# CrystalSixone/VLN-MAGIC

Hardware: AMD Instinct MI355X
Metric: trajectory-steps/sec (whole node), MAGIC-S R2R pretrain (higher is better)
Workload: dtype bf16

## Files before the change

### include/magic_hip.h

```cpp
#ifndef MAGIC_HIP_H
#define MAGIC_HIP_H
#ifdef __cplusplus
extern "C" {
#endif

#define MAGIC_OK 0
#define MAGIC_ERR_ARG (-1)
#define MAGIC_ERR_LAUNCH (-2)
#define MAGIC_ERR_UNSUPPORTED (-3)

int magic_abi_version(void);
int magic_build_id(char* out, int len);
int magic_device_info(int* cu_count, int* clock_khz, char* arch, int arch_len);

int magic_gemm(int dtype, int layout, int batch, int nh, int M, int N, int K,
               const void* A, int lda, long long sAb, long long sAh,
               const void* B, int ldb, long long sBb, long long sBh,
               void* C, int ldc, long long sCb, long long sCh, int c_f32, int accumulate,
               const float* bias, int epilogue, const void* aux, int ldaux,
               const void* residual, int ldr, void* C2, int ldc2,
               float alpha, int splitk, float* bias_grad, void* stream);
int magic_gemm_set_big(int mode);
#define MAGIC_GEMM_FORM_PLAIN 0x1
#define MAGIC_GEMM_FORM_XCD 0x2
// ... 184 lines not shown
int magic_mlm_eval_ws_need(int dtype, int nm, int V, int H);
int magic_mlm_eval(int dtype, int nm, int V, int H, const void* hm, const void* W, int ldw, const float* bias,
                   const int* labels, int ignore_index, void* ws, float* loss_row, int* hit_row, void* stream);
int magic_eval_rows(int dtype, int M, int N, const void* logits, int ld, const int* labels, int ignore_index,
                    const float* targets, int ldt, float* loss_row, int* hit_row, void* stream);
int magic_cfp_eval(int dtype, int B, int H, const void* a, const void* txt, float temperature,
                   float* loss_row, int* hit_row, void* stream);
int magic_eval_accum(int M, const float* loss_row, const int* hit_row, void* acc, int slot, void* stream);

int magic_csr_gather(int dtype, int n_out, int H, const void* src, const int* ptr, const int* idx, const float* w,
                     void* out, int accumulate, void* stream);
int magic_pano_fuse_fwd(int dtype, int N, int V, int H, const void* x, const int* lens, const float* wf, const float* bf,
                        void* fused, float* probs, const void* P, int nh, int inner, float* pmean, void* stream);
typedef struct {
  int B, K, Vp, use_gate;
  const float *g_raw, *l_raw, *fuse_raw; const unsigned char *gmask, *lmask; const int* fsrc; const unsigned char* bwmask;
  float *gl, *ll, *fl;
  const int *glab, *llab; int ignore_index; float coef;
  float *rows, *dgl, *dll, *dfl;
  const float* t_fused; float w_rate; int pad_; float* w_out;
  float T, kd_norm, kd_coef, pad2_; const float* kd_coef_dev; float* kd_rows;
} magic_sap_loss_params;
int magic_sap_fuse_loss(const void* params, int nbytes, void* stream);
int magic_pano_fuse_bwd_blocks(int N);
int magic_pano_fuse_bwd(int dtype, int N, int V, int H, const void* x, const float* probs, const float* wf, const void* dfused,
                        void* dx, float* dwf, float* dbf, void* stream);
int magic_sap_fuse_fwd(int B, int K, int Vp, const float* g_raw, const float* l_raw, const float* fuse_raw,
                       const unsigned char* gmask, const unsigned char* lmask, const int* fsrc, const unsigned char* bwmask,
                       int use_gate, float* gl, float* ll, float* fl, void* stream);
int magic_sap_fuse_bwd(int B, int K, int Vp, const float* g_raw, const float* l_raw, const float* fuse_raw,
                       const unsigned char* gmask, const unsigned char* lmask, const int* fsrc, const unsigned char* bwmask,
                       int use_gate, const float* dgl, const float* dll, const float* dfl,
                       float* dg_raw, float* dl_raw, float* dfuse_raw, void* stream);

int magic_step_rng(unsigned long long base_seed, unsigned* counter, float rw_temp, int* seed_out, float* rw_out, float* zero_me,
                   float* scale_state, float growth, float backoff, int interval, void* stream);
int magic_seed_scale(const float* scale_dev);
int magic_loss_assemble(const float* rows, int n_rows, const float* row_w, float row_scale, const float* kd_rows, int n_kd,
                        float* slots, const float* rw, float alpha, int has_kd, float* out, void* stream);

int magic_rowgate_fwd(int dtype, int M, int H, int mode, const void* x, const void* e, const float* wx, const float* we,
                      const float* b0, const float* b1, float* out_s, void* out, float* gsave, void* stream);
int magic_rowgate_bwd(int dtype, int M, int H, int mode, const void* x, const void* e, const float* wx, const float* we, const float* gsave,
                      const float* dy, const void* dout, void* dx, void* de, float* dwx, float* dwe, float* db0, float* db1, void* stream);

int magic_sumsq(long long n, const float* g, float* out, void* stream);
int magic_adamw(long long n, float* p, float* g, float* m, float* v, void* shadow, int shadow_dtype,
                float lr, float b1, float b2, float eps, float wd, float step_size,
                const float* sumsq, float max_norm, float gscale, const float* lr_ss, long long n_decay, int zero_grad,
                unsigned* overflow, float* scale_state, int* sched_step, int decay_first, void* stream);
int magic_sumsq_sched(long long n, const float* g, float* out, int* step, float lr0, int warmup, int total, float b1, float b2,
                      float* lr_ss, void* stream);
int magic_sched_step(int* step, float lr0, int warmup, int total, float b1, float b2, float* lr_ss, float* zero_me, void* stream);
int magic_cast(int dtype16, int to16, long long n, const void* x, void* y, void* stream);
int magic_add_n(int dtype, long long n, int count, const void* const* xs, void* y, void* stream);
int magic_add(int dtype, long long n, const void* x, void* y, void* stream);
int magic_dact(int dtype, int kind, long long n, const void* dy, const void* z, void* dz, void* stream);

int magic_view_gather(int dtype, int Np, int V, int D, const void* table, int n_viewpoints, const int* vp_row,
                      const int* order, void* out, void* stream);

int magic_set_f32_mfma(int mode);
int magic_get_f32_mfma(void);

typedef struct {
  const void* Wqkv; const float* bqkv; const void* Wo; const float* bo; const float* g1; const float* be1;
// ... 81 lines not shown
```

### vln-magic_amd/host/heads.py

```python
import contextlib

import torch

from . import lib as _lib
from . import makd_pretrain as KD
from . import model_pretrain as MP
from . import ops as O
from .config import cfg_get
from .engine import rup


def cls_fwd(n, prefix, X, M, lda=None):
    l1 = n.lin(prefix + "net.0.weight")
    Y = O.linear_fwd(X, l1.W, l1.b, M, epilogue=2, lda=lda)
    return Y, cls_tail(n, prefix, Y, M)


def cls_tail(n, prefix, Y, M):
    ln, l2 = n.ln(prefix + "net.2"), n.lin(prefix + "net.3.weight")
    logit = n.new(M, dtype=torch.float32)
    O.lndot_fwd(Y, M, n.H, ln.g, ln.b, n.eps, l2.Wm, l2.b, logit)
    return logit


def cls_bwd(n, prefix, X, Y, dlogit, M, d_acc, lda=None):
    H = n.H
    l1, ln, l2 = n.lin(prefix + "net.0.weight"), n.ln(prefix + "net.2"), n.lin(prefix + "net.3.weight")
    dZ = n.new(M, H)
    O.lndot_bwd(Y, M, H, ln.g, ln.b, n.eps, l2.Wm, dlogit, dZ, ln.dg, ln.db, l2.dW, l2.db)
    O.linear_dw(dZ, X, l1.dW, l1.db, M, ldb=lda)
    O.linear_dx(dZ, l1.W, M, out=d_acc, residual=d_acc, ldc=lda)


def gate_fuse_bwd(n, prefix, c, df, B, K, Vp, d_gmap, d_vp, grouped):
    H = n.H
    f1, fln, f2 = n.lin(prefix + "sap_fuse_linear.net.0.weight"), n.ln(prefix + "sap_fuse_linear.net.2"), n.lin(prefix + "sap_fuse_linear.net.3.weight")
    dZ = n.new(B, H)
    O.lndot_bwd(c.Yf, B, H, fln.g, fln.b, n.eps, f2.Wm, df, dZ, fln.dg, fln.db, f2.dW, f2.db)
    O.linear_dw(dZ, c.glob.out, f1.dW, f1.db, B, N=H, K=H, ldb=K * H, ldc=2 * H)
    O.linear_dw(dZ, c.loc.out, f1.dW[:, H:], None, B, N=H, K=H, ldb=Vp * H, ldc=2 * H)
    with _lib.group() if grouped else contextlib.nullcontext():
        O.linear_dx(dZ, f1.W, B, out=d_gmap, residual=d_gmap, ldb=2 * H, ldc=K * H, N=H, K=H)
        O.linear_dx(dZ, f1.W[:, H:], B, out=d_vp, residual=d_vp, ldb=2 * H, ldc=Vp * H, N=H, K=H)


def _relu(x):
    return O.dact(x, x, 2, out=x)


def _sizes(m, c):
    p = c.plan
    return m.net, p, p["B"], p["L"], p["K"], p["Vp"], m.net.H


class Head:
    gpos = vpos = True

    def dx_rows(self, plan):
        return 0

    def kd_sample_w(self, m, c, t, kdl):
        return None

    def kd_predict(self, m, c, t, T, w, coef):
        return None


class Mlm(Head):
    vpos = False

    def cross(self, m, c, o):
        n, plan, B, L, K, Vp, H = _sizes(m, c)
        l2v_args = ("global", plan, c.txt_out, L, plan["txt_mask"], plan["lens"]["txt"], plan["txt_tokens"],
                    c.gin.out, K, plan["gmap_mask"], plan["lens"]["gmap"], plan["gmap_nodes"])
        c.l2v = n.cross_fwd_fused([l2v_args])[0] if n.xenc_ok(L, K) else n.cross_fwd(*l2v_args, dist=None)
        o["gmap_embeds"], o["gmap_attns"] = c.l2v.out, c.l2v.P

    def head(self, m, c, o, compute_loss, metrics):
        n, plan, B, L, K, Vp, H = _sizes(m, c)
        nm = plan["n_mask"]
# ... 177 lines not shown
        o.update(gmap_embeds=c.glob.out, gmap_attns=c.glob.P, vp_embeds=c.loc.out, vp_attns=c.loc.P)

    def kd_streams(self, c):
        p = c.plan
        return {"global": (c.glob.out, c.glob.P, p["K"], p["L"], c.glob.ldp, c.d_gmap, "K", "L"),
                "local": (c.loc.out, c.loc.P, p["Vp"], p["L"], c.loc.ldp, c.d_vp, None, "L")}

    def _encoders_bwd(self, m, c):
        n, plan = m.net, c.plan
        d_txt2 = c.d_txt2
        one = not getattr(c, "islands", None) and n.nodes_pano_ok(plan, gin=c.gin, vin=c.vin)
        fold = None
        if n.rbw_ok():
            (d_gin, d_vin), fold = n.cross_stacks_bwd([(c.glob, c.d_gmap, c.d_txt, c.dP_g), (c.loc, c.d_vp, c.d_txt, c.dP_l)], defer_fold=one)
        else:
            d_gin, d_vin = m._par(lambda: n.cross_bwd(c.glob, c.d_gmap, c.d_txt, c.dP_g),
                                  lambda: n.cross_bwd(c.loc, c.d_vp, d_txt2, c.dP_l))
            if one:
                fold = (c.d_txt, [d_txt2])
            else:
                O.add_(c.d_txt, d_txt2)
        if one:
            n.nodes_pano_bwd(plan, c.pano, c.gin, d_gin, c.vin, d_vin, c.d_pano, c.d_fused, add=fold)
            c.pano_head_done = True
        else:
            n.nodes_in_bwd(plan, c.gin, d_gin, c.vin, d_vin, c.d_pano, c.d_fused)


class Sap(_Glocal):
    def head(self, m, c, o, compute_loss, metrics):
        n, plan, B, L, K, Vp, H = _sizes(m, c)
        use_gate = bool(cfg_get(m.config, "glocal_fuse"))
        g1, l1_ = n.lin("global_sap_head.net.0.weight"), n.lin("local_sap_head.net.0.weight")
        with _lib.group():
            c.Yg = O.linear_fwd(c.glob.out, g1.W, g1.b, B * K, epilogue=2)
            c.Yl = O.linear_fwd(c.loc.out, l1_.W, l1_.b, B * Vp, epilogue=2)
            if use_gate:
                f1 = n.lin("sap_fuse_linear.net.0.weight")
                tmp = O.linear_fwd(c.glob.out, f1.W, None, B, lda=K * H, ldb=2 * H, K=H)
        c.g_raw = cls_tail(n, "global_sap_head.", c.Yg, B * K)
        c.l_raw = cls_tail(n, "local_sap_head.", c.Yl, B * Vp)
        if use_gate:
            c.Yf = O.linear_fwd(c.loc.out, f1.W[:, H:], f1.b, B, lda=Vp * H, ldb=2 * H, K=H, residual=tmp, epilogue=0)
            _relu(c.Yf)
            fln, f2 = n.ln("sap_fuse_linear.net.2"), n.lin("sap_fuse_linear.net.3.weight")
            c.fuse_raw = n.new(B, dtype=torch.float32)
            O.lndot_fwd(c.Yf, B, H, fln.g, fln.b, n.eps, f2.Wm, f2.b, c.fuse_raw)
        else:
            c.fuse_raw = n.zeros(B, dtype=torch.float32)
        c.use_gate = use_gate
        c.gl, c.ll, c.fl = n.new(B, K, dtype=torch.float32), n.new(B, Vp, dtype=torch.float32), n.new(B, K, dtype=torch.float32)
        c.sap_fused = bool(compute_loss and O.SAP_LOSS_FUSED and K <= 512 and Vp <= 128)
        if not c.sap_fused:
            O.sap_fuse_fwd(B, K, Vp, c.g_raw, c.l_raw, c.fuse_raw, plan["gmask"], plan["lmask"], plan["fsrc"], plan["bwmask"],
                           use_gate, c.gl, c.ll, c.fl)
        o.update(global_logits=c.gl, local_logits=c.ll, fused_logits=c.fl)

    def rows(self, plan):
        B = plan["B"]
        return [B * plan["K"], B * plan["Vp"], B * plan["L"]]

    def loss(self, m, c, o, zz, scg, kd):
        n, plan, B, L, K, Vp, H = _sizes(m, c)
        train = m.store.requires_grad
        c.d_gmap, c.d_vp, c.d_txt2 = zz(B * K, H), zz(B * Vp, H), zz(B * L, H)
        c.rows = n.new(3, B, dtype=torch.float32)
        c.dgl, c.dll, c.dfl = (n.new(B, K, dtype=torch.float32), n.new(B, Vp, dtype=torch.float32), n.new(B, K, dtype=torch.float32)) \
            if train else (None, None, None)
        ga, la = plan["global_act_labels"], plan["local_act_labels"]
        c.sap_w = c.kdrows = None
        if c.sap_fused:
            kdl = kd.kdl if kd else None
            hard = bool(kd and kdl.get("teacher_sample_hard_mining", False))
            pred = bool(kd and "predict" in kdl["kdl_tasks"])
            if hard:
                c.sap_w = n.new(B, dtype=torch.float32)
            if pred:
                c.kdrows = n.new(B, dtype=torch.float32)
            if kd:
                rwd = KD.rw_device(m, kd.rw)
            O.sap_fuse_loss(B, K, Vp, c.g_raw, c.l_raw, c.fuse_raw, plan["gmask"], plan["lmask"], plan["fsrc"], plan["bwmask"], c.use_gate,
                            c.gl, c.ll, c.fl, ga, la, scg / B, c.rows, dgl=c.dgl, dll=c.dll, dfl=c.dfl,
                            t_fused=kd.t["fused_logits"] if (hard or pred) else None,
                            w_rate=float(kdl["t_sample_preprocess_exp_decay"]) if hard else 0.0, w_out=c.sap_w,
                            T=float(kdl["kd_temperature"]) if kd else 1.0, kd_norm=(1.0 / B if hard else 1.0 / (B * K)),
                            kd_coef=kd.alpha * kd.gs if kd else 0.0, kd_coef_dev=rwd[4:5] if pred else None, kd_rows=c.kdrows)
        else:
            O.ce_rows(c.gl, B, K, K, ga, coef=scg / B, loss_row=c.rows[0], dlogits=c.dgl, ldd=K)
            O.ce_rows(c.ll, B, Vp, Vp, la, coef=scg / B, loss_row=c.rows[1], dlogits=c.dll, ldd=Vp)
            O.ce_rows(c.fl, B, K, K, ga, coef=scg / B, loss_row=c.rows[2], dlogits=c.dfl, ldd=K)
        return c.rows, None, 1.0 / B

    def kd_sample_w(self, m, c, t, kdl):
        if c.sap_w is not None:
            return c.sap_w
        n, plan = m.net, c.plan
        w = n.new(plan["B"], dtype=torch.float32)
        O.ce_rows(t["fused_logits"], plan["B"], plan["K"], plan["K"], plan["global_act_labels"], w_out=w,
                  w_rate=float(kdl["t_sample_preprocess_exp_decay"]))
        return w

    def kd_predict(self, m, c, t, T, w, coef):
        if not c.sap_fused:
            B, K = c.plan["B"], c.plan["K"]
            c.kdrows = m.net.new(B, dtype=torch.float32)
            O.kd_rows(c.fl, t["fused_logits"], B, K, K, T, w=w, norm=(1.0 / B if w is not None else 1.0 / (B * K)),
                      coef=coef[0], coef_dev=coef[1], loss_row=c.kdrows, ds=c.dfl, accumulate=True)
        return c.kdrows

    def backward(self, m, c):
        n, plan, B, L, K, Vp, H = _sizes(m, c)
        dg, dl, df = n.new(B, K, dtype=torch.float32), n.new(B, Vp, dtype=torch.float32), n.new(B, dtype=torch.float32)
        O.sap_fuse_bwd(B, K, Vp, c.g_raw, c.l_raw, c.fuse_raw, plan["gmask"], plan["lmask"], plan["fsrc"], plan["bwmask"],
                       c.use_gate, c.dgl, c.dll, c.dfl, dg, dl, df)
        heads = []
        for prefix, X, Y, dlogit, M, d_acc in (("global_sap_head.", c.glob.out, c.Yg, dg, B * K, c.d_gmap),
                                               ("local_sap_head.", c.loc.out, c.Yl, dl, B * Vp, c.d_vp)):
            l1, ln, l2 = n.lin(prefix + "net.0.weight"), n.ln(prefix + "net.2"), n.lin(prefix + "net.3.weight")
            dZh = n.new(M, H)
            O.lndot_bwd(Y, M, H, ln.g, ln.b, n.eps, l2.Wm, dlogit, dZh, ln.dg, ln.db, l2.dW, l2.db)
            O.linear_dw(dZh, X, l1.dW, l1.db, M)
            heads.append((dZh, l1, M, d_acc))
        with _lib.group():
            for dZh, l1, M, d_acc in heads:
                O.linear_dx(dZh, l1.W, M, out=d_acc, residual=d_acc)
        if c.use_gate:
            gate_fuse_bwd(n, "", c, df, B, K, Vp, c.d_gmap, c.d_vp, grouped=True)
        self._encoders_bwd(m, c)

    def metrics(self, m, c, block, temperature):
        plan = c.plan
        B, K, Vp = plan["B"], plan["K"], plan["Vp"]
        ga, la = plan["global_act_labels"], plan["local_act_labels"]
        for slot, (x, N, lab) in enumerate(((c.gl, K, ga), (c.ll, Vp, la), (c.fl, K, ga))):
            O.eval_accum(*O.eval_rows(x, B, N, N, labels=lab), B, block, slot)

    def result(self, m, c, o, batch):
        return dict(global_logits=c.gl, local_logits=c.ll, fused_logits=c.fl,
                    global_act_labels=m._dev(batch["global_act_labels"]), local_act_labels=m._dev(batch["local_act_labels"]))


class Cfp(_Glocal):
    def head(self, m, c, o, compute_loss, metrics):
        n, plan, B, L, K, Vp, H = _sizes(m, c)
# ... 96 lines not shown
```

### vln-magic_amd/host/ops.py

```python
import contextlib
import ctypes as C
import os

import torch

from . import lanes
from . import lib as L

FLOPS = {"total": 0.0, "gemm": 0.0, "linear_ln": 0.0, "attn": 0.0, "enc": 0.0, "enabled": False}
BYTES = {"dw": 0.0, "dw_launches": 0}


def _flops(f, fam):
    if FLOPS["enabled"]:
        FLOPS["total"] += f
        FLOPS[fam] = FLOPS.get(fam, 0.0) + f


def _count(m, n, k, batch=1, fam="gemm"):
    _flops(2.0 * m * n * k * batch, fam)


_SUPPORTED = {}

# ... 1146 lines not shown
def pano_fuse_bwd(x, probs, wf, dfused, dx, dwf, dbf, N, V, H):
    dwf, dbf = _fuse_part(N, H, dwf, dbf, x.device)
    L.call("magic_pano_fuse_bwd", L.dt(x.dtype), N, V, H, L.P(x), L.P(probs), L.P(wf), L.P(dfused), L.P(dx), L.P(dwf), L.P(dbf),
           L.stream())


def sap_fuse_fwd(B, K, Vp, g_raw, l_raw, fuse_raw, gmask, lmask, fsrc, bwmask, use_gate, gl, ll, fl):
    L.call("magic_sap_fuse_fwd", B, K, Vp, L.P(g_raw), L.P(l_raw), L.P(fuse_raw), L.P(gmask), L.P(lmask), L.P(fsrc), L.P(bwmask),
           1 if use_gate else 0, L.P(gl), L.P(ll), L.P(fl), L.stream())


SAP_LOSS_FUSED = not os.environ.get("MAGIC_NO_SAP_LOSS_FUSED")


def sap_fuse_loss(B, K, Vp, g_raw, l_raw, fuse_raw, gmask, lmask, fsrc, bwmask, use_gate, gl, ll, fl, glab, llab, coef, rows, *, dgl=None, dll=None,
                  dfl=None, ignore_index=-100, t_fused=None, w_rate=0.0, w_out=None, T=1.0, kd_norm=0.0, kd_coef=0.0, kd_coef_dev=None, kd_rows=None):
    _chk(glab.dtype == torch.int32 and llab.dtype == torch.int32 and rows.dtype == torch.float32 and rows.numel() >= 3 * B, "sap_fuse_loss labels int32, rows fp32 [3, B]")
    _chk(t_fused is None or (t_fused.dtype == torch.float32 and t_fused.is_contiguous() and tuple(t_fused.shape) == (B, K)), "sap_fuse_loss teacher logits fp32 [B, K]")
    P = L.SapLossParams()
    P.B, P.K, P.Vp, P.use_gate = B, K, Vp, 1 if use_gate else 0
    for k, v in (("g_raw", g_raw), ("l_raw", l_raw), ("fuse_raw", fuse_raw), ("gmask", gmask), ("lmask", lmask), ("fsrc", fsrc), ("bwmask", bwmask),
                 ("gl", gl), ("ll", ll), ("fl", fl), ("glab", glab), ("llab", llab), ("rows", rows), ("dgl", dgl), ("dll", dll), ("dfl", dfl),
                 ("t_fused", t_fused), ("w_out", w_out), ("kd_coef_dev", kd_coef_dev), ("kd_rows", kd_rows)):
        setattr(P, k, L.P(v))
    P.ignore_index, P.coef, P.w_rate, P.T, P.kd_norm, P.kd_coef = int(ignore_index), float(coef), float(w_rate), float(T), float(kd_norm), float(kd_coef)
    L.call("magic_sap_fuse_loss", C.addressof(P), C.sizeof(P), L.stream())


def sap_fuse_bwd(B, K, Vp, g_raw, l_raw, fuse_raw, gmask, lmask, fsrc, bwmask, use_gate, dgl, dll, dfl, dg_raw, dl_raw, dfuse_raw):
    L.call("magic_sap_fuse_bwd", B, K, Vp, L.P(g_raw), L.P(l_raw), L.P(fuse_raw), L.P(gmask), L.P(lmask), L.P(fsrc), L.P(bwmask),
           1 if use_gate else 0, L.P(dgl), L.P(dll), L.P(dfl), L.P(dg_raw), L.P(dl_raw), L.P(dfuse_raw), L.stream())


def step_rng(base_seed, counter, rw_temp, seed_out=None, rw_out=None, zero_me=None, scale_state=None, growth=2.0, backoff=0.5, interval=2000):
    L.call("magic_step_rng", int(base_seed) & 0xFFFFFFFFFFFFFFFF, L.P(counter), float(rw_temp), L.P(seed_out), L.P(rw_out), L.P(zero_me),
           L.P(scale_state), float(growth), float(backoff), int(interval), L.stream())


def rowgate_fwd(mode, x, M, H, wx, *, e=None, we=None, b0=None, b1=None, out_s=None, out=None, gsave=None):
    L.call("magic_rowgate_fwd", L.dt(x.dtype), M, H, mode, L.P(x), L.P(e), L.P(wx), L.P(we), L.P(b0), L.P(b1), L.P(out_s), L.P(out), L.P(gsave), L.stream())


def rowgate_bwd(mode, x, M, H, wx, *, e=None, we=None, gsave=None, dy=None, dout=None, dx=None, de=None, dwx=None, dwe=None, db0=None, db1=None):
    L.call("magic_rowgate_bwd", L.dt(x.dtype), M, H, mode, L.P(x), L.P(e), L.P(wx), L.P(we), L.P(gsave), L.P(dy), L.P(dout), L.P(dx), L.P(de),
           L.P(dwx), L.P(dwe), L.P(db0), L.P(db1), L.stream())


def seed_scale(scale_state):
    L.call("magic_seed_scale", L.P(scale_state))


def loss_assemble(rows, row_w, row_scale, kd_rows, slots, rw, alpha, has_kd, out):
    _chk(rows.dtype == torch.float32 and rows.is_contiguous() and out.dtype == torch.float32 and out.numel() >= 13, "loss_assemble layout")
    L.call("magic_loss_assemble", L.P(rows), rows.numel(), L.P(row_w), float(row_scale), L.P(kd_rows), kd_rows.numel() if kd_rows is not None else 0,
           L.P(slots), L.P(rw), float(alpha), 1 if has_kd else 0, L.P(out), L.stream())
    return out


def sumsq(g, out):
    L.call("magic_sumsq", g.numel(), L.P(g), L.P(out), L.stream())


def sumsq_sched(g, out, step, lr0, warmup, total, b1, b2, lr_ss):
    _chk(step.numel() >= 2 and step.dtype == torch.int32, "schedule step words: int32[2] {global_step, optimizer state step}")
    L.call("magic_sumsq_sched", g.numel(), L.P(g), L.P(out), L.P(step), float(lr0), int(warmup), int(total), float(b1), float(b2), L.P(lr_ss), L.stream())

# ... 43 lines not shown
```

Baseline: 197,800.

## Fuse SAP head MLPs, LayerNorm, logits and backward into single kernels

Adds a forward kernel that computes the global, local and gate SAP head linear+ReLU, LayerNorm and dot-product logits in one launch, grouping blocks per head. Adds a backward kernel per batch row and side that folds the SAP fuse-loss gradient, LayerNorm/dot backward and the dX GEMM against LDS-staged weights. Weight-gradient GEMMs stay separate. The aim is to remove many small launches and intermediate round trips, at the cost of heavy register/LDS use and a one-block-per-sample backward with limited parallelism.

```diff
diff --git a/include/magic_hip.h b/include/magic_hip.h
--- a/include/magic_hip.h
+++ b/include/magic_hip.h
@@ -240,6 +240,23 @@
                        const unsigned char* gmask, const unsigned char* lmask, const int* fsrc, const unsigned char* bwmask,
                        int use_gate, const float* dgl, const float* dll, const float* dfl,
                        float* dg_raw, float* dl_raw, float* dfuse_raw, void* stream);
+int magic_sap_heads_fwd_supported(int dtype, int K, int Vp, int H);
+int magic_sap_heads_bwd_supported(int dtype, int K, int Vp, int H);
+int magic_sap_heads_fwd(int dtype, int B, int K, int Vp, int H, int use_gate, float eps, const void* Xg, const void* Xl,
+                        const void* Wg, const float* bg, const float* gam_g, const float* bet_g, const float* w2g, const float* b2g,
+                        const void* Wl, const float* bl, const float* gam_l, const float* bet_l, const float* w2l, const float* b2l,
+                        const void* Wf, const float* bf, const float* gam_f, const float* bet_f, const float* w2f, const float* b2f,
+                        void* Yg, void* Yl, void* Yf, float* g_raw, float* l_raw, float* fuse_raw, void* stream);
+int magic_sap_heads_bwd(int dtype, int B, int K, int Vp, int H, int use_gate, float eps,
+                        const float* g_raw, const float* l_raw, const float* fuse_raw, const unsigned char* gmask, const unsigned char* lmask,
+                        const int* fsrc, const unsigned char* bwmask, const float* dgl, const float* dll, const float* dfl,
+                        const void* Yg, const void* Wg, const float* gam_g, const float* bet_g, const float* w2g, void* dZg,
+                        float* dgam_g, float* dbet_g, float* dw2g, float* db2g,
+                        const void* Yl, const void* Wl, const float* gam_l, const float* bet_l, const float* w2l, void* dZl,
+                        float* dgam_l, float* dbet_l, float* dw2l, float* db2l,
+                        const void* Yf, const void* Wf, const float* gam_f, const float* bet_f, const float* w2f, void* dZf,
+                        float* dgam_f, float* dbet_f, float* dw2f, float* db2f,
+                        void* d_gmap, void* d_vp, float* part, void* stream);
 
 int magic_step_rng(unsigned long long base_seed, unsigned* counter, float rw_temp, int* seed_out, float* rw_out, float* zero_me,
                    float* scale_state, float growth, float backoff, int interval, void* stream);
diff --git a/vln-magic_amd/csrc/sapheads.hip b/vln-magic_amd/csrc/sapheads.hip
--- /dev/null
+++ b/vln-magic_amd/csrc/sapheads.hip
@@ -0,0 +1,432 @@
+#include "common.hpp"
+
+#define SH_NT 256
+#define SH_R 16
+#define SH_KMAX 512
+#define SH_VMAX 128
+
+template <typename T> __device__ __forceinline__ void sh_ld2(const T* p, float& a, float& b) {
+  a = (float)p[0]; b = (float)p[1];
+}
+template <typename T> __device__ __forceinline__ void sh_st2(T* p, float a, float b) {
+  typedef __attribute__((ext_vector_type(2))) T v2;
+  v2 v; v[0] = (T)a; v[1] = (T)b; *(v2*)p = v;
+}
+
+struct SapHeadF {
+  const void* X; const void* W; const float* b; const float* gamma; const float* beta; const float* w2; const float* b2;
+  void* Y; float* raw; int M; long long lda;
+};
+struct SapHeadsFwd { SapHeadF h[3]; const void* X2; long long lda2; int start[4]; float eps; int zero_fuse; };
+
+template <typename Hh, int NIT>
+__global__ __launch_bounds__(SH_NT) void sap_heads_fwd_kernel(SapHeadsFwd p) {
+  constexpr int H = 128 * NIT, NT = 2 * NIT, YP = H + 8;
+  __shared__ __attribute__((aligned(16))) Hh sY[SH_R * YP];
+  typedef h16x8<Hh> v8;
+  int hi = 0;
+  while (hi < 2 && (int)blockIdx.x >= p.start[hi + 1]) ++hi;
+  const SapHeadF& q = p.h[hi];
+  const int tid = threadIdx.x, lane = tid & 63, wid = tid >> 6;
+  const int r0 = ((int)blockIdx.x - p.start[hi]) * SH_R, M = q.M;
+  const bool gate = hi == 2;
+  const int ldw = gate ? 2 * H : H, n0 = wid * (H / 4), ar = r0 + (lane & 15);
+  if (p.zero_fuse && blockIdx.x == 0)
+    for (int i = tid; i < p.h[2].M; i += SH_NT) p.h[2].raw[i] = 0.f;
+
+  f32x4 acc[NT];
+  auto product = [&](const Hh* __restrict__ X, long long lda, const Hh* __restrict__ W) {
+#pragma unroll
+    for (int j = 0; j < NT; ++j) acc[j] = (f32x4){0.f, 0.f, 0.f, 0.f};
+    v8 a[H / 32], b[H / 32][NT];
+#pragma unroll
+    for (int ks = 0; ks < H / 32; ++ks) {
+#pragma unroll
+      for (int e = 0; e < 8; ++e) a[ks][e] = (Hh)0.0f;
+      if (ar < M) a[ks] = *(const v8*)(X + (long long)ar * lda + ks * 32 + 8 * (lane >> 4));
+#pragma unroll
+      for (int j = 0; j < NT; ++j) b[ks][j] = *(const v8*)(W + (long long)(n0 + 16 * j + (lane & 15)) * ldw + ks * 32 + 8 * (lane >> 4));
+    }
+#pragma unroll
+    for (int ks = 0; ks < H / 32; ++ks)
+#pragma unroll
+      for (int j = 0; j < NT; ++j) acc[j] = mfma16(a[ks], b[ks][j], acc[j]);
+  };
+  float bv[NT];
+#pragma unroll
+  for (int j = 0; j < NT; ++j) bv[j] = q.b[n0 + 16 * j + (lane & 15)];
+  float gmv[2 * NIT], btv[2 * NIT], w2v[2 * NIT];
+#pragma unroll
+  for (int i = 0; i < 2 * NIT; ++i) {
+    const int c = (i >> 1) * 128 + lane * 2 + (i & 1);
+    gmv[i] = q.gamma[c]; btv[i] = q.beta[c]; w2v[i] = q.w2[c];
+  }
+  const float b2v = q.b2[0];
+  product((const Hh*)q.X, q.lda, (const Hh*)q.W);
+  if (!gate) {
+#pragma unroll
+    for (int j = 0; j < NT; ++j)
+#pragma unroll
+      for (int r = 0; r < 4; ++r)
+        sY[(4 * (lane >> 4) + r) * YP + n0 + 16 * j + (lane & 15)] = from_f<Hh>(fmaxf(acc[j][r] * 1.f + bv[j], 0.f));
+  } else {
+    float t1[NT][4];
+#pragma unroll
+    for (int j = 0; j < NT; ++j)
+#pragma unroll
+      for (int r = 0; r < 4; ++r) t1[j][r] = to_f(from_f<Hh>(acc[j][r] * 1.f + 0.f));
+    product((const Hh*)p.X2, p.lda2, (const Hh*)q.W + H);
+#pragma unroll
+    for (int j = 0; j < NT; ++j)
+#pragma unroll
+      for (int r = 0; r < 4; ++r) {
+        const Hh y = from_f<Hh>((acc[j][r] * 1.f + bv[j]) + t1[j][r]);
+        sY[(4 * (lane >> 4) + r) * YP + n0 + 16 * j + (lane & 15)] = to_f(y) > 0.f ? y : from_f<Hh>(0.f);
+      }
+  }
+  __syncthreads();
+  Hh* __restrict__ Y = (Hh*)q.Y;
+  const float eps = p.eps;
+  for (int rr = 0; rr < 4; ++rr) {
+    const int lr = 4 * wid + rr, row = r0 + lr;
+    if (row >= M) break;
+    float x[2 * NIT];
+    float s = 0.f;
+#pragma unroll
+    for (int it = 0; it < NIT; ++it) { sh_ld2<Hh>(sY + lr * YP + it * 128 + lane * 2, x[2 * it], x[2 * it + 1]); s += x[2 * it] + x[2 * it + 1]; }
+#pragma unroll
+    for (int it = 0; it < NIT; ++it) sh_st2<Hh>(Y + (long long)row * H + it * 128 + lane * 2, x[2 * it], x[2 * it + 1]);
+    const float mean = wave_sum(s) / H;
+    float qq = 0.f;
+#pragma unroll
+    for (int it = 0; it < NIT; ++it) { float a = x[2 * it] - mean, b = x[2 * it + 1] - mean; qq += a * a + b * b; }
+    const float rstd = rsqrtf(wave_sum(qq) / H + eps);
+    float d = 0.f;
+#pragma unroll
+    for (int it = 0; it < NIT; ++it)
+      d += ((x[2 * it] - mean) * rstd * gmv[2 * it] + btv[2 * it]) * w2v[2 * it] + ((x[2 * it + 1] - mean) * rstd * gmv[2 * it + 1] + btv[2 * it + 1]) * w2v[2 * it + 1];
+    d = wave_sum(d);
+    if (lane == 0) q.raw[row] = d + b2v;
+  }
+}
+
+struct SapHeadB {
+  const void* Y; const void* W; const float* gamma; const float* beta; const float* w2; void* dZ;
+  float* dgamma; float* dbeta; float* dw2; float* db2;
+};
+struct SapHeadsBwd {
+  SapHeadB h[3];
+  int B, K, Vp, use_gate; float eps;
+  const float *g_raw, *l_raw, *fuse_raw; const unsigned char *gmask, *lmask; const int* fsrc; const unsigned char* bwmask;
+  const float *dgl, *dll, *dfl;
+  void* d_gmap; void* d_vp; float* part;
+};
+
+static size_t sap_heads_bwd_lds(int H) {
+  return (size_t)H * (H + 8) * 2 + (size_t)SH_R * (H + 8) * 2 + (size_t)2 * H * 2 + (size_t)(SH_KMAX + SH_VMAX + 4) * 4 +
+         (H == 128 ? (size_t)H * (H + 8) * 2 : 0);
+}
+
+template <typename Hh, int NIT>
+__global__ __launch_bounds__(SH_NT) void sap_heads_bwd_kernel(SapHeadsBwd p) {
+  constexpr int H = 128 * NIT, NT = 2 * NIT, WP = H + 8;
+  extern __shared__ __attribute__((aligned(16))) unsigned char shb_smem[];
+  Hh* const sW = (Hh*)shb_smem;
+  float* const red = (float*)shb_smem;
+  Hh* const sD = sW + H * WP;
+  Hh* const sStop = sD + SH_R * WP;
+  float* const sdg = (float*)(sStop + 2 * H);
+  float* const sdl = sdg + SH_KMAX;
+  float* const smisc = sdl + SH_VMAX;
+  Hh* const sW2 = (Hh*)(smisc + 4);
+  typedef h16x8<Hh> v8;
+  const int tid = threadIdx.x, lane = tid & 63, wid = tid >> 6;
+  const int b = blockIdx.x >> 1, side = blockIdx.x & 1, K = p.K, Vp = p.Vp;
+  const bool gate = p.use_gate != 0;
+  const float eps = p.eps;
+  const Hh* const Wside = (const Hh*)p.h[side].W;
+  const Hh* const Wgate = p.use_gate ? (const Hh*)p.h[2].W + side * H : nullptr;
+
+  auto load_W = [&](Hh* dst, const Hh* __restrict__ W, const int ldw) {
+    for (int i = tid; i < H * (H / 8); i += SH_NT) {
+      const int row = i / (H / 8), cv = i % (H / 8);
+      *(v8*)(dst + row * WP + cv * 8) = *(const v8*)(W + (long long)row * ldw + cv * 8);
+    }
+  };
+  constexpr int WR = NIT == 1 ? H * (H / 8) / SH_NT : 1;
+  v8 wreg[2 * WR];
+  if constexpr (NIT == 1) {
+#pragma unroll
+    for (int i = 0; i < WR; ++i) {
+      const int c = tid + SH_NT * i, row = c / (H / 8), cv = c % (H / 8);
+      wreg[i] = *(const v8*)(Wside + (long long)row * H + cv * 8);
+      if (gate) wreg[WR + i] = *(const v8*)(Wgate + (long long)row * 2 * H + cv * 8);
+    }
+  }
+
+  {
+    const float fw = gate ? 1.f / (1.f + __expf(-p.fuse_raw[b])) : 0.5f;
+    if (tid < 64) {
+      for (int j = tid; j < Vp; j += 64) sdl[j] = p.lmask[b * Vp + j] ? p.dll[b * Vp + j] : 0.f;
+      if (tid == 0) smisc[0] = 0.f;
+    }
+    __syncthreads();
+    float dfw = 0.f;
+    if (tid < 64)
+      for (int k = tid; k < K; k += 64) {
+        const bool ok = p.gmask[b * K + k];
+        const float dg = ok ? (p.dgl[b * K + k] + p.dfl[b * K + k]) : 0.f;
+        sdg[k] = dg * fw;
+        dfw += dg * p.g_raw[b * K + k];
+        if (ok) {
+          const int s = p.fsrc[b * K + k];
+          const float d = p.dfl[b * K + k];
+          if (s >= 0 && s < Vp) atomicAdd(&sdl[s], d); else if (s == -2) atomicAdd(&smisc[0], d);
+        }
+      }
+    __syncthreads();
+    if (tid < 64) {
+      const float sbw = smisc[0];
+      for (int j = tid; j < Vp; j += 64) {
+        float d = sdl[j];
+        if (p.bwmask[b * Vp + j]) d += sbw;
+        if (!p.lmask[b * Vp + j]) d = 0.f;
+        sdl[j] = d * (1.f - fw);
+        dfw -= d * p.l_raw[b * Vp + j];
+      }
+      dfw = wave_sum(dfw);
+      if (tid == 0) smisc[1] = gate ? dfw * fw * (1.f - fw) : 0.f;
+    }
+    __syncthreads();
+  }
+  if constexpr (NIT == 1) {
+#pragma unroll
+    for (int i = 0; i < WR; ++i) {
+      const int c = tid + SH_NT * i, row = c / (H / 8), cv = c % (H / 8);
+      *(v8*)(sW + row * WP + cv * 8) = wreg[i];
+      if (gate) *(v8*)(sW2 + row * WP + cv * 8) = wreg[WR + i];
+    }
+  } else {
+    load_W(sW, Wside, H);
+  }
+
+  auto head = [&](const int hidx, const Hh* sWi, const long long row0, const int n, const float* sdlogit, Hh* __restrict__ dacc, const bool keep,
+                  const bool write) {
+    const SapHeadB& q = p.h[hidx];
+    const Hh* __restrict__ Y = (const Hh*)q.Y;
+    Hh* __restrict__ dZ = (Hh*)q.dZ;
+    float gmv[2 * NIT], btv[2 * NIT], w2v[2 * NIT];
+#pragma unroll
+    for (int i = 0; i < 2 * NIT; ++i) {
+      const int c = (i >> 1) * 128 + lane * 2 + (i & 1);
+      gmv[i] = q.gamma[c]; btv[i] = q.beta[c]; w2v[i] = q.w2[c];
+    }
+    float ag[2 * NIT], ab[2 * NIT], aw[2 * NIT];
+#pragma unroll
+    for (int i = 0; i < 2 * NIT; ++i) { ag[i] = 0.f; ab[i] = 0.f; aw[i] = 0.f; }
+    float adb = 0.f;
+    const int ntile = (n + SH_R - 1) / SH_R, n0 = wid * (H / 4);
+    for (int t = 0; t < ntile; ++t) {
+      float xr[4][2 * NIT];
+#pragma unroll
+      for (int rr = 0; rr < 4; ++rr) {
+        const int kk = SH_R * t + 4 * wid + rr;
+#pragma unroll
+        for (int it = 0; it < NIT; ++it) {
+          xr[rr][2 * it] = 0.f; xr[rr][2 * it + 1] = 0.f;
+          if (kk < n) sh_ld2<Hh>(Y + (row0 + kk) * H + it * 128 + lane * 2, xr[rr][2 * it], xr[rr][2 * it + 1]);
+        }
+      }
+      Hh old[NT][4];
+#pragma unroll
+      for (int j = 0; j < NT; ++j)
+#pragma unroll
+        for (int r = 0; r < 4; ++r) {
+          const int kk = SH_R * t + 4 * (lane >> 4) + r, col = n0 + 16 * j + (lane & 15);
+          old[j][r] = from_f<Hh>(0.f);
+          if (kk < n) old[j][r] = (kk == 0 && !keep) ? sStop[col] : dacc[(long long)kk * H + col];
+        }
+#pragma unroll
+      for (int rr = 0; rr < 4; ++rr) {
+        const int lr = 4 * wid + rr, kk = SH_R * t + lr;
+        if (kk >= n) {
+#pragma unroll
+          for (int it = 0; it < NIT; ++it) sh_st2<Hh>(sD + lr * WP + it * 128 + lane * 2, 0.f, 0.f);
+          continue;
+        }
+        const long long row = row0 + kk;
+        float x[2 * NIT];
+        float s = 0.f;
+#pragma unroll
+        for (int it = 0; it < NIT; ++it) { x[2 * it] = xr[rr][2 * it]; x[2 * it + 1] = xr[rr][2 * it + 1]; s += x[2 * it] + x[2 * it + 1]; }
+        const float mean = wave_sum(s) / H;
+        float qq = 0.f;
+#pragma unroll
+        for (int it = 0; it < NIT; ++it) { float a = x[2 * it] - mean, c = x[2 * it + 1] - mean; qq += a * a + c * c; }
+        const float rstd = rsqrtf(wave_sum(qq) / H + eps);
+        const float dl = sdlogit[kk];
+        adb += dl;
+        float g[2 * NIT], xh[2 * NIT];
+        float s1 = 0.f, s2 = 0.f;
+#pragma unroll
+        for (int it = 0; it < NIT; ++it) {
+#pragma unroll
+          for (int e = 0; e < 2; ++e) {
+            const int i = 2 * it + e;
+            xh[i] = (x[i] - mean) * rstd;
+            const float dln = dl * w2v[i];
+            aw[i] += dl * (xh[i] * gmv[i] + btv[i]);
+            ag[i] += dln * xh[i]; ab[i] += dln;
+            g[i] = dln * gmv[i];
+            s1 += g[i]; s2 += g[i] * xh[i];
+          }
+        }
+        const float m1 = wave_sum(s1) / H, m2 = wave_sum(s2) / H;
+#pragma unroll
+        for (int it = 0; it < NIT; ++it) {
+          const float da = x[2 * it] > 0.f ? rstd * (g[2 * it] - m1 - xh[2 * it] * m2) : 0.f;
+          const float dbv = x[2 * it + 1] > 0.f ? rstd * (g[2 * it + 1] - m1 - xh[2 * it + 1] * m2) : 0.f;
+          if (write) sh_st2<Hh>(dZ + row * H + it * 128 + lane * 2, da, dbv);
+          sh_st2<Hh>(sD + lr * WP + it * 128 + lane * 2, da, dbv);
+        }
+      }
+      __syncthreads();
+      {
+        f32x4 acc[NT];
+#pragma unroll
+        for (int j = 0; j < NT; ++j) acc[j] = (f32x4){0.f, 0.f, 0.f, 0.f};
+#pragma unroll
+        for (int ks = 0; ks < H / 32; ++ks) {
+          const v8 a = frag_kc<Hh>(sD, WP, 0, ks * 32, lane);
+          v8 bb[NT];
+#pragma unroll
+          for (int j = 0; j < NT; ++j) bb[j] = frag_oc<Hh>(sWi, WP, n0 + 16 * j, ks * 32, lane);
+#pragma unroll
+          for (int j = 0; j < NT; ++j) acc[j] = mfma16(a, bb[j], acc[j]);
+        }
+#pragma unroll
+        for (int j = 0; j < NT; ++j)
+#pragma unroll
+          for (int r = 0; r < 4; ++r) {
+            const int kk = SH_R * t + 4 * (lane >> 4) + r, col = n0 + 16 * j + (lane & 15);
+            if (kk < n) {
+              const Hh out = from_f<Hh>(acc[j][r] * 1.f + to_f(old[j][r]));
+              dacc[(long long)kk * H + col] = out;
+              if (kk == 0 && keep) sStop[col] = out;
+            }
+          }
+      }
+      __syncthreads();
+    }
+    if (!write) return;
+#pragma unroll
+    for (int it = 0; it < NIT; ++it) {
+      const int c = it * 128 + lane * 2;
+      red[(0 * 4 + wid) * H + c] = ag[2 * it]; red[(0 * 4 + wid) * H + c + 1] = ag[2 * it + 1];
+      red[(1 * 4 + wid) * H + c] = ab[2 * it]; red[(1 * 4 + wid) * H + c + 1] = ab[2 * it + 1];
+      red[(2 * 4 + wid) * H + c] = aw[2 * it]; red[(2 * 4 + wid) * H + c + 1] = aw[2 * it + 1];
+    }
+    if (lane == 0) red[12 * H + wid] = adb;
+    __syncthreads();
+    if (p.part) {
+      float* row = p.part + ((long long)b * (gate ? 3 : 2) + hidx) * (3 * H + 1);
+      for (int c = tid; c < H; c += SH_NT) {
+        row[c] = red[c] + red[H + c] + red[2 * H + c] + red[3 * H + c];
+        row[H + c] = red[4 * H + c] + red[5 * H + c] + red[6 * H + c] + red[7 * H + c];
+        row[2 * H + c] = red[8 * H + c] + red[9 * H + c] + red[10 * H + c] + red[11 * H + c];
+      }
+      if (tid == 0) row[3 * H] = red[12 * H] + red[12 * H + 1] + red[12 * H + 2] + red[12 * H + 3];
+    } else {
+      for (int c = tid; c < H; c += SH_NT) {
+        atomicAdd(q.dgamma + c, red[c] + red[H + c] + red[2 * H + c] + red[3 * H + c]);
+        atomicAdd(q.dbeta + c, red[4 * H + c] + red[5 * H + c] + red[6 * H + c] + red[7 * H + c]);
+        atomicAdd(q.dw2 + c, red[8 * H + c] + red[9 * H + c] + red[10 * H + c] + red[11 * H + c]);
+      }
+      if (tid == 0) atomicAdd(q.db2, red[12 * H] + red[12 * H + 1] + red[12 * H + 2] + red[12 * H + 3]);
+    }
+    __syncthreads();
+  };
+
+  Hh* const rows = side ? (Hh*)p.d_vp + (long long)b * Vp * H : (Hh*)p.d_gmap + (long long)b * K * H;
+  head(side, sW, side ? (long long)b * Vp : (long long)b * K, side ? Vp : K, side ? sdl : sdg, rows, true, true);
+  if (gate) {
+    if constexpr (NIT != 1) load_W(sW, Wgate, 2 * H);
+    head(2, NIT == 1 ? sW2 : sW, b, 1, smisc + 1, rows, false, side == 1);
+  }
+}
+
+static bool sap_heads_shape_ok(int dtype, int B, int K, int Vp, int H) {
+  return dtype_is16(dtype) && (H == 128 || H == 256) && B > 0 && K > 0 && K <= SH_KMAX && Vp > 0 && Vp <= SH_VMAX &&
+         (long long)B * K * H <= 0x7FFFFFFFll && (long long)B * Vp * H <= 0x7FFFFFFFll;
+}
+static bool al16(const void* q) { return ((uintptr_t)q & 15) == 0; }
+
+extern "C" int magic_sap_heads_fwd_supported(int dtype, int K, int Vp, int H) { return sap_heads_shape_ok(dtype, 1, K, Vp, H) ? 1 : 0; }
+extern "C" int magic_sap_heads_bwd_supported(int dtype, int K, int Vp, int H) { return sap_heads_shape_ok(dtype, 1, K, Vp, H) ? 1 : 0; }
+
+extern "C" int magic_sap_heads_fwd(int dtype, int B, int K, int Vp, int H, int use_gate, float eps, const void* Xg, const void* Xl,
+                                   const void* Wg, const float* bg, const float* gam_g, const float* bet_g, const float* w2g, const float* b2g,
+                                   const void* Wl, const float* bl, const float* gam_l, const float* bet_l, const float* w2l, const float* b2l,
+                                   const void* Wf, const float* bf, const float* gam_f, const float* bet_f, const float* w2f, const float* b2f,
+                                   void* Yg, void* Yl, void* Yf, float* g_raw, float* l_raw, float* fuse_raw, void* stream) {
+  if (!sap_heads_shape_ok(dtype, B, K, Vp, H)) return MAGIC_ERR_ARG;
+  if (!Xg || !Xl || !Wg || !bg || !gam_g || !bet_g || !w2g || !b2g || !Wl || !bl || !gam_l || !bet_l || !w2l || !b2l || !Yg || !Yl || !g_raw || !l_raw ||
+      !fuse_raw) return MAGIC_ERR_ARG;
+  if (use_gate && (!Wf || !bf || !gam_f || !bet_f || !w2f || !b2f || !Yf)) return MAGIC_ERR_ARG;
+  if (!al16(Xg) || !al16(Xl) || !al16(Wg) || !al16(Wl) || (use_gate && !al16(Wf)) || ((uintptr_t)Yg & 3) || ((uintptr_t)Yl & 3) || ((uintptr_t)Yf & 3)) return MAGIC_ERR_ARG;
+  SapHeadsFwd p;
+  p.h[0] = SapHeadF{Xg, Wg, bg, gam_g, bet_g, w2g, b2g, Yg, g_raw, B * K, (long long)H};
+  p.h[1] = SapHeadF{Xl, Wl, bl, gam_l, bet_l, w2l, b2l, Yl, l_raw, B * Vp, (long long)H};
+  p.h[2] = SapHeadF{Xg, Wf, bf, gam_f, bet_f, w2f, b2f, Yf, fuse_raw, B, (long long)K * H};
+  p.X2 = Xl; p.lda2 = (long long)Vp * H;
+  p.eps = eps; p.zero_fuse = use_gate ? 0 : 1;
+  p.start[0] = 0;
+  p.start[1] = (B * K + SH_R - 1) / SH_R;
+  p.start[2] = p.start[1] + (B * Vp + SH_R - 1) / SH_R;
+  p.start[3] = p.start[2] + (use_gate ? (B + SH_R - 1) / SH_R : 0);
+  dim3 grid(p.start[3]), block(SH_NT);
+  hipStream_t st = (hipStream_t)stream;
+  if (H == 128) DISPATCH_H(dtype, hipLaunchKernelGGL((sap_heads_fwd_kernel<TY, 1>), grid, block, 0, st, p));
+  else DISPATCH_H(dtype, hipLaunchKernelGGL((sap_heads_fwd_kernel<TY, 2>), grid, block, 0, st, p));
+  return launch_status();
+}
+
+extern "C" int magic_sap_heads_bwd(int dtype, int B, int K, int Vp, int H, int use_gate, float eps,
+                                   const float* g_raw, const float* l_raw, const float* fuse_raw, const unsigned char* gmask, const unsigned char* lmask,
+                                   const int* fsrc, const unsigned char* bwmask, const float* dgl, const float* dll, const float* dfl,
+                                   const void* Yg, const void* Wg, const float* gam_g, const float* bet_g, const float* w2g, void* dZg,
+                                   float* dgam_g, float* dbet_g, float* dw2g, float* db2g,
+                                   const void* Yl, const void* Wl, const float* gam_l, const float* bet_l, const float* w2l, void* dZl,
+                                   float* dgam_l, float* dbet_l, float* dw2l, float* db2l,
+                                   const void* Yf, const void* Wf, const float* gam_f, const float* bet_f, const float* w2f, void* dZf,
+                                   float* dgam_f, float* dbet_f, float* dw2f, float* db2f,
+                                   void* d_gmap, void* d_vp, float* part, void* stream) {
+  if (!sap_heads_shape_ok(dtype, B, K, Vp, H)) return MAGIC_ERR_ARG;
+  if (!g_raw || !l_raw || !fuse_raw || !gmask || !lmask || !fsrc || !bwmask || !dgl || !dll || !dfl || !d_gmap || !d_vp) return MAGIC_ERR_ARG;
+  if (!Yg || !Wg || !gam_g || !bet_g || !w2g || !dZg || !Yl || !Wl || !gam_l || !bet_l || !w2l || !dZl) return MAGIC_ERR_ARG;
+  if (use_gate && (!Yf || !Wf || !gam_f || !bet_f || !w2f || !dZf)) return MAGIC_ERR_ARG;
+  if (!part && (!dgam_g || !dbet_g || !dw2g || !db2g || !dgam_l || !dbet_l || !dw2l || !db2l || (use_gate && (!dgam_f || !dbet_f || !dw2f || !db2f)))) return MAGIC_ERR_ARG;
+  if (!al16(Wg) || !al16(Wl) || (use_gate && !al16(Wf)) || ((uintptr_t)Yg & 3) || ((uintptr_t)Yl & 3) || ((uintptr_t)Yf & 3) || ((uintptr_t)dZg & 3) ||
+      ((uintptr_t)dZl & 3) || ((uintptr_t)dZf & 3) || ((uintptr_t)d_gmap & 1) || ((uintptr_t)d_vp & 1)) return MAGIC_ERR_ARG;
+  SapHeadsBwd p;
+  p.h[0] = SapHeadB{Yg, Wg, gam_g, bet_g, w2g, dZg, dgam_g, dbet_g, dw2g, db2g};
+  p.h[1] = SapHeadB{Yl, Wl, gam_l, bet_l, w2l, dZl, dgam_l, dbet_l, dw2l, db2l};
+  p.h[2] = SapHeadB{Yf, Wf, gam_f, bet_f, w2f, dZf, dgam_f, dbet_f, dw2f, db2f};
+  p.B = B; p.K = K; p.Vp = Vp; p.use_gate = use_gate ? 1 : 0; p.eps = eps;
+  p.g_raw = g_raw; p.l_raw = l_raw; p.fuse_raw = fuse_raw; p.gmask = gmask; p.lmask = lmask; p.fsrc = fsrc; p.bwmask = bwmask;
+  p.dgl = dgl; p.dll = dll; p.dfl = dfl; p.d_gmap = d_gmap; p.d_vp = d_vp; p.part = part;
+  const size_t lds = sap_heads_bwd_lds(H);
+  static bool attr = false;
+  if (!attr) {
+    (void)hipFuncSetAttribute((const void*)sap_heads_bwd_kernel<bf16, 1>, hipFuncAttributeMaxDynamicSharedMemorySize, (int)sap_heads_bwd_lds(128));
+    (void)hipFuncSetAttribute((const void*)sap_heads_bwd_kernel<f16, 1>, hipFuncAttributeMaxDynamicSharedMemorySize, (int)sap_heads_bwd_lds(128));
+    (void)hipFuncSetAttribute((const void*)sap_heads_bwd_kernel<bf16, 2>, hipFuncAttributeMaxDynamicSharedMemorySize, (int)sap_heads_bwd_lds(256));
+    (void)hipFuncSetAttribute((const void*)sap_heads_bwd_kernel<f16, 2>, hipFuncAttributeMaxDynamicSharedMemorySize, (int)sap_heads_bwd_lds(256));
+    attr = true;
+  }
+  dim3 grid(2 * B), block(SH_NT);
+  hipStream_t st = (hipStream_t)stream;
+  if (H == 128) DISPATCH_H(dtype, hipLaunchKernelGGL((sap_heads_bwd_kernel<TY, 1>), grid, block, lds, st, p));
+  else DISPATCH_H(dtype, hipLaunchKernelGGL((sap_heads_bwd_kernel<TY, 2>), grid, block, lds, st, p));
+  return launch_status();
+}
diff --git a/vln-magic_amd/host/heads.py b/vln-magic_amd/host/heads.py
--- a/vln-magic_amd/host/heads.py
+++ b/vln-magic_amd/host/heads.py
@@ -1,4 +1,5 @@
 import contextlib
+import os
 
 import torch
 
@@ -46,6 +47,15 @@
 
 def _relu(x):
     return O.dact(x, x, 2, out=x)
+
+
+def _sap_heads_on(ok, x, K, Vp, H):
+    return not os.environ.get("MAGIC_NO_SAP_HEADS") and ok(x.dtype, K, Vp, H)
+
+
+def _sap_params(n, use_gate):
+    return [(n.lin(p + "net.0.weight"), n.ln(p + "net.2"), n.lin(p + "net.3.weight"))
+            for p in ("global_sap_head.", "local_sap_head.") + (("sap_fuse_linear.",) if use_gate else ())]
 
 
 def _sizes(m, c):
@@ -289,6 +299,13 @@
         n, plan, B, L, K, Vp, H = _sizes(m, c)
         use_gate = bool(cfg_get(m.config, "glocal_fuse"))
         g1, l1_ = n.lin("global_sap_head.net.0.weight"), n.lin("local_sap_head.net.0.weight")
+        if _sap_heads_on(O.sap_heads_fwd_ok, c.glob.out, K, Vp, H):
+            c.Yg, c.Yl, c.Yf = n.new(B * K, H), n.new(B * Vp, H), (n.new(B, H) if use_gate else None)
+            c.g_raw, c.l_raw, c.fuse_raw = n.new(B * K, dtype=torch.float32), n.new(B * Vp, dtype=torch.float32), n.new(B, dtype=torch.float32)
+            O.sap_heads_fwd(B, K, Vp, H, n.eps, c.glob.out, c.loc.out,
+                            [(l1.W, l1.b, ln.g, ln.b, l2.Wm, l2.b) for l1, ln, l2 in _sap_params(n, use_gate)],
+                            (c.Yg, c.Yl, c.Yf), (c.g_raw, c.l_raw, c.fuse_raw))
+            return self._fuse(m, c, o, compute_loss, use_gate)
         with _lib.group():
             c.Yg = O.linear_fwd(c.glob.out, g1.W, g1.b, B * K, epilogue=2)
             c.Yl = O.linear_fwd(c.loc.out, l1_.W, l1_.b, B * Vp, epilogue=2)
@@ -305,6 +322,10 @@
             O.lndot_fwd(c.Yf, B, H, fln.g, fln.b, n.eps, f2.Wm, f2.b, c.fuse_raw)
         else:
             c.fuse_raw = n.zeros(B, dtype=torch.float32)
+        self._fuse(m, c, o, compute_loss, use_gate)
+
+    def _fuse(self, m, c, o, compute_loss, use_gate):
+        n, plan, B, L, K, Vp, H = _sizes(m, c)
         c.use_gate = use_gate
         c.gl, c.ll, c.fl = n.new(B, K, dtype=torch.float32), n.new(B, Vp, dtype=torch.float32), n.new(B, K, dtype=torch.float32)
         c.sap_fused = bool(compute_loss and O.SAP_LOSS_FUSED and K <= 512 and Vp <= 128)
@@ -367,6 +388,20 @@
 
     def backward(self, m, c):
         n, plan, B, L, K, Vp, H = _sizes(m, c)
+        if _sap_heads_on(O.sap_heads_bwd_ok, c.Yg, K, Vp, H):
+            par = _sap_params(n, c.use_gate)
+            dZ = [n.new(M, H) for M in (B * K, B * Vp, B)[:len(par)]]
+            O.sap_heads_bwd(B, K, Vp, H, n.eps, c.g_raw, c.l_raw, c.fuse_raw, plan["gmask"], plan["lmask"], plan["fsrc"], plan["bwmask"],
+                            c.dgl, c.dll, c.dfl,
+                            [(Y, l1.W, ln.g, ln.b, l2.Wm, dz, ln.dg, ln.db, l2.dW, l2.db) for (l1, ln, l2), Y, dz in zip(par, (c.Yg, c.Yl, c.Yf), dZ)],
+                            c.d_gmap, c.d_vp)
+            O.linear_dw(dZ[0], c.glob.out, par[0][0].dW, par[0][0].db, B * K)
+            O.linear_dw(dZ[1], c.loc.out, par[1][0].dW, par[1][0].db, B * Vp)
+            if c.use_gate:
+                f1 = par[2][0]
+                O.linear_dw(dZ[2], c.glob.out, f1.dW, f1.db, B, N=H, K=H, ldb=K * H, ldc=2 * H)
+                O.linear_dw(dZ[2], c.loc.out, f1.dW[:, H:], None, B, N=H, K=H, ldb=Vp * H, ldc=2 * H)
+            return self._encoders_bwd(m, c)
         dg, dl, df = n.new(B, K, dtype=torch.float32), n.new(B, Vp, dtype=torch.float32), n.new(B, dtype=torch.float32)
         O.sap_fuse_bwd(B, K, Vp, c.g_raw, c.l_raw, c.fuse_raw, plan["gmask"], plan["lmask"], plan["fsrc"], plan["bwmask"],
                        c.use_gate, c.dgl, c.dll, c.dfl, dg, dl, df)
diff --git a/vln-magic_amd/host/ops.py b/vln-magic_amd/host/ops.py
--- a/vln-magic_amd/host/ops.py
+++ b/vln-magic_amd/host/ops.py
@@ -1202,6 +1202,64 @@
            1 if use_gate else 0, L.P(dgl), L.P(dll), L.P(dfl), L.P(dg_raw), L.P(dl_raw), L.P(dfuse_raw), L.stream())
 
 
+def sap_heads_fwd_ok(dtype, K, Vp, H):
+    return dtype in L.HALF and bool(_supported("magic_sap_heads_fwd_supported", L.dt(dtype), int(K), int(Vp), int(H)))
+
+
+def sap_heads_bwd_ok(dtype, K, Vp, H):
+    return dtype in L.HALF and bool(_supported("magic_sap_heads_bwd_supported", L.dt(dtype), int(K), int(Vp), int(H)))
+
+
+def _sap_head_chk(W, H, cols, vecs, what):
+    _chk(tuple(W.shape) == (H, cols) and W.stride(1) == 1 and W.stride(0) == cols, what + " weight")
+    _chk(all(v.dtype == torch.float32 and v.is_contiguous() and v.numel() >= n for v, n in vecs), what + " fp32 parameters")
+
+
+def sap_heads_fwd(B, K, Vp, H, eps, Xg, Xl, heads, Ys, raws):
+    use_gate = len(heads) == 3
+    _chk(len(heads) in (2, 3) and len(Ys) == 3 and len(raws) == 3, "sap_heads_fwd heads")
+    _chk(Xg.dtype == Xl.dtype and Xg.is_contiguous() and Xl.is_contiguous() and Xg.numel() >= B * K * H and Xl.numel() >= B * Vp * H, "sap_heads_fwd rows")
+    args = []
+    for i, (W, b, g, bt, w2, b2) in enumerate(heads):
+        _chk(W.dtype == Xg.dtype, "sap_heads_fwd weight dtype")
+        _sap_head_chk(W, H, 2 * H if i == 2 else H, ((b, H), (g, H), (bt, H), (w2, H), (b2, 1)), "sap_heads_fwd")
+        args += [L.P(W), L.P(b), L.P(g), L.P(bt), L.P(w2), L.P(b2)]
+    args += [None] * (18 - len(args))
+    for Y, raw, M in zip(Ys, raws, (B * K, B * Vp, B)):
+        _chk(raw.dtype == torch.float32 and raw.is_contiguous() and raw.numel() >= M, "sap_heads_fwd logits fp32")
+        _chk(Y is None or (Y.dtype == Xg.dtype and Y.is_contiguous() and Y.numel() >= M * H), "sap_heads_fwd Y")
+    _chk(Ys[0] is not None and Ys[1] is not None and (Ys[2] is not None or not use_gate), "sap_heads_fwd Y")
+    _count(B * (K + Vp + (2 if use_gate else 0)), H, H)
+    L.call("magic_sap_heads_fwd", L.dt(Xg.dtype), B, K, Vp, H, 1 if use_gate else 0, float(eps), L.P(Xg), L.P(Xl), *args,
+           L.P(Ys[0]), L.P(Ys[1]), L.P(Ys[2]), L.P(raws[0]), L.P(raws[1]), L.P(raws[2]), L.stream())
+
+
+def sap_heads_bwd(B, K, Vp, H, eps, g_raw, l_raw, fuse_raw, gmask, lmask, fsrc, bwmask, dgl, dll, dfl, heads, d_gmap, d_vp):
+    use_gate = len(heads) == 3
+    _chk(len(heads) in (2, 3), "sap_heads_bwd heads")
+    _chk(all(t.dtype == torch.float32 and t.is_contiguous() for t in (g_raw, l_raw, fuse_raw, dgl, dll, dfl)), "sap_heads_bwd fp32 logits and gradients")
+    _chk(g_raw.numel() >= B * K and dgl.numel() >= B * K and dfl.numel() >= B * K and l_raw.numel() >= B * Vp and dll.numel() >= B * Vp and fuse_raw.numel() >= B,
+         "sap_heads_bwd logit extents")
+    _chk(gmask.numel() >= B * K and fsrc.numel() >= B * K and lmask.numel() >= B * Vp and bwmask.numel() >= B * Vp and gmask.element_size() == 1
+         and lmask.element_size() == 1 and bwmask.element_size() == 1 and fsrc.dtype == torch.int32, "sap_heads_bwd masks")
+    dt_ = d_gmap.dtype
+    _chk(d_vp.dtype == dt_ and d_gmap.is_contiguous() and d_vp.is_contiguous() and d_gmap.numel() >= B * K * H and d_vp.numel() >= B * Vp * H, "sap_heads_bwd accumulators")
+    part, fields, args, stride = None, [], [], 3 * H + 1
+    for i, (Y, W, g, bt, w2, dZ, dg, dbt, dw2, db2) in enumerate(heads):
+        M = (B * K, B * Vp, B)[i]
+        _chk(Y.dtype == W.dtype == dZ.dtype == dt_ and Y.is_contiguous() and dZ.is_contiguous() and Y.numel() >= M * H and dZ.numel() >= M * H, "sap_heads_bwd Y / dZ")
+        _sap_head_chk(W, H, 2 * H if i == 2 else H, ((g, H), (bt, H), (w2, H), (dg, H), (dbt, H), (dw2, H), (db2, 1)), "sap_heads_bwd")
+        args += [L.P(Y), L.P(W), L.P(g), L.P(bt), L.P(w2), L.P(dZ), L.P(dg), L.P(dbt), L.P(dw2), L.P(db2)]
+        o = i * stride
+        fields += [(o, H, dg.reshape(-1)), (o + H, H, dbt.reshape(-1)), (o + 2 * H, H, dw2.reshape(-1)), (o + 3 * H, 1, db2.reshape(-1))]
+    args += [None] * (30 - len(args))
+    if part_ok(H):
+        part = _part_block(B, len(heads) * stride, d_gmap.device, fields)
+    _count(B * (K + Vp + (2 if use_gate else 0)), H, H)
+    L.call("magic_sap_heads_bwd", L.dt(dt_), B, K, Vp, H, 1 if use_gate else 0, float(eps), L.P(g_raw), L.P(l_raw), L.P(fuse_raw), L.P(gmask), L.P(lmask),
+           L.P(fsrc), L.P(bwmask), L.P(dgl), L.P(dll), L.P(dfl), *args, L.P(d_gmap), L.P(d_vp), L.P(part), L.stream())
+
+
 def step_rng(base_seed, counter, rw_temp, seed_out=None, rw_out=None, zero_me=None, scale_state=None, growth=2.0, backoff=0.5, interval=2000):
     L.call("magic_step_rng", int(base_seed) & 0xFFFFFFFFFFFFFFFF, L.P(counter), float(rw_temp), L.P(seed_out), L.P(rw_out), L.P(zero_me),
            L.P(scale_state), float(growth), float(backoff), int(interval), L.stream())
```

New measurement: 199,100 (median of 6 runs). No clear change (+0.7%).
